# zxhuang1698/ShapeClipper

Measured on AMD Instinct MI355X. Metric: train-step images/sec (Pix3D cfg, bs32/GPU), higher is better.
Workload: dtype f32 (bf16x3-split MFMA, fp32 accumulate)

## Files before the change

### include/shapeclipper_hip.h

```cpp
#ifndef SHAPECLIPPER_HIP_H
#define SHAPECLIPPER_HIP_H
#include <stdint.h>
#ifdef __cplusplus
extern "C" {
#endif

int sc_chamfer3d_forward(const float* xyz1, const float* xyz2, float* dist1, float* dist2,
                         int32_t* idx1, int32_t* idx2, int b, int n, int m, void* stream);

int sc_chamfer3d_forward_split(const float* xyz1, const float* xyz2, float* dist1, float* dist2,
                               int32_t* idx1, int32_t* idx2, int b, int n, int m, int nsplit,
                               void* workspace, void* stream);

long long sc_chamfer3d_grid_workspace_bytes(int b, int n, int m);
int sc_chamfer3d_forward_grid(const float* xyz1, const float* xyz2, float* dist1, float* dist2,
                              int32_t* idx1, int32_t* idx2, int b, int n, int m, void* workspace, void* stream);

int sc_chamfer3d_backward(const float* xyz1, const float* xyz2, float* gradxyz1, float* gradxyz2,
                          const float* graddist1, const float* graddist2, const int32_t* idx1,
                          const int32_t* idx2, int b, int n, int m, void* stream);

long long sc_chamfer3d_backward_ordered_workspace_bytes(int b, int n, int m);
int sc_chamfer3d_backward_ordered_chunk(void);
int sc_chamfer3d_backward_ordered(const float* xyz1, const float* xyz2, float* gradxyz1, float* gradxyz2,
// ... 372 lines not shown

long long sc_conv3x3s2_bd_pack_floats(int cin, int cout, int hw);
long long sc_conv3x3s2_bd_workspace_floats(int hw);
int sc_conv3x3s2_bd_pack(const float* w, float* w_pack, int cin, int cout, int hw, void* stream);
int sc_conv3x3s2_backward_data(const float* gy, const float* w_pack, float* gx, float* workspace, int batch, int cin, int cout, int hw,
                               void* stream);
int sc_conv3x3s2_wgrad(const float* gy, const float* x, float* dw, float* workspace, int batch, int cin, int cout, int hw, void* stream);
long long sc_conv3x3s2_pack_floats(int cin, int cout, int hw);
long long sc_conv3x3s2_workspace_floats(int hw);
int sc_conv3x3s2_forward(const float* x, const float* w_pack, float* out, float* workspace, int batch, int cin, int cout, int hw,
                         void* stream);

long long sc_conv3x3_wgrad_workspace_floats(int cin, int cout);
int sc_conv3x3_wgrad(const float* gy, const float* x, float* dw, float* workspace, int batch, int cin, int cout, int hw, void* stream);
int sc_conv3x3_wgrad_split(const float* gy, const float* x, float* dw, float* workspace, int batch, int cin, int cout, int hw, void* stream);

long long sc_conv_stem_wgrad_workspace_floats(void);
int sc_conv_stem_forward(const float* x, const float* w, float* out, int batch, void* stream);
int sc_conv_stem_wgrad(const float* gy, const float* x, float* dw, float* workspace, int batch, void* stream);

long long sc_conv1x1s2_wgrad_workspace_floats(int cin, int cout);
int sc_conv1x1s2_forward(const float* x, const float* w, float* out, int batch, int cin, int cout, int hin, void* stream);
int sc_conv1x1s2_backward_data(const float* gy, const float* w, float* gx, int batch, int cin, int cout, int hin, void* stream);
int sc_conv1x1s2_wgrad(const float* gy, const float* x, float* dw, float* workspace, int batch, int cin, int cout, int hin, void* stream);

typedef struct sc_block_args {
    const float *x, *pf1, *pf2, *pb1, *pb2;
    const float *g1, *b1, *g2, *b2;
    float *rm1, *rv1, *rm2, *rv2;
    int64_t *nt1, *nt2;
// ... 57 lines not shown
```

### shapeclipper_amd/_lib.py

```python
from __future__ import annotations

import ctypes
import os
import re
import threading
from typing import Optional

import torch

_HERE = os.path.dirname(os.path.abspath(__file__))
LIB_PATH = os.environ.get("SHAPECLIPPER_HIP_LIB") or os.path.join(_HERE, "lib", "libshapeclipper_hip.so")

HEADER_PATH = os.path.join(_HERE, os.pardir, "include", "shapeclipper_hip.h")
_CTYPES = {"int": ctypes.c_int, "long long": ctypes.c_longlong, "float": ctypes.c_float, "double": ctypes.c_double}


def read_signatures(text):
    text = re.sub(r"/\*.*?\*/|//[^\n]*", " ", text, flags=re.S)
    text = re.sub(r"^[ \t]*#.*$", " ", text, flags=re.M)
    text = re.sub(r"typedef struct sc_block_args \{.*?\} sc_block_args", " ", text, flags=re.S)
    text = re.sub(r'extern "C" \{|\}', " ", text)
    sigs = {}
    for decl in filter(None, (" ".join(d.split()) for d in text.split(";"))):
        m = re.fullmatch(r"(int|long long) (sc_\w+)\((.*)\)", decl)
        if m is None:
            raise RuntimeError("shapeclipper_amd: include/shapeclipper_hip.h: unrecognised declaration %r" % decl)
        params = [] if m.group(3) == "void" else m.group(3).split(",")
        try:
            args = [ctypes.c_void_p if "*" in p else _CTYPES[" ".join(w for w in p.split()[:-1] if w != "const")] for p in params]
        except KeyError:
            raise RuntimeError("shapeclipper_amd: include/shapeclipper_hip.h: unrecognised parameter type in %r" % decl) from None
        sigs[m.group(2)] = (_CTYPES[m.group(1)], args)
    return sigs


with open(HEADER_PATH) as _f:
    SIGNATURES = read_signatures(_f.read())
SYMBOLS = tuple(n for n, (res, _) in SIGNATURES.items() if res is ctypes.c_int)
SYMBOLS_OTHER = tuple(n for n, (res, _) in SIGNATURES.items() if res is ctypes.c_longlong)

_lib: Optional[ctypes.CDLL] = None

TIMING = None
TIMING_SKIP = ("sc_sdf_stream_pack", "sc_sdf_stream_pack_bytes", "sc_rgb_composite_backward_fused_parts", "sc_rgb_composite_backward_fused_partial_floats", "sc_latent_bias_forward", "sc_latent_bias_backward", "sc_set_reserved_cus", "sc_grid_cus", "sc_chamfer3d_backward_ordered_chunk","sc_conv3x3_release_tables", "sc_linear_bn_supported", "sc_linear_bn_forward", "sc_linear_bn_backward", "sc_linear_backward_data", "sc_bn_splits", "sc_isosurface_blocks_per_image", "sc_marching_cubes_mesh_vertex_blocks_per_image", "sc_bn_act_forward", "sc_bn_act_backward", "sc_bn_relu_pool_forward", "sc_bn_relu_pool_backward",
               "sc_conv3x3_forward", "sc_conv3x3_forward_split", "sc_conv3x3_forward_add", "sc_conv3x3_wgrad", "sc_conv3x3_wgrad_split", "sc_conv3x3_pack", "sc_conv3x3_pack_multi", "sc_conv3x3_pack_multi_units",
               "sc_conv_stem_forward", "sc_conv_stem_wgrad", "sc_conv1x1s2_forward", "sc_conv1x1s2_backward_data", "sc_conv1x1s2_wgrad",
               "sc_conv3x3s2_forward", "sc_conv3x3s2_bd_pack", "sc_conv3x3s2_backward_data", "sc_conv3x3s2_wgrad", "sc_conv3x3_tile_channels", "sc_conv3x3_tile_channels_split",
               "sc_basic_block_forward", "sc_basic_block_backward")

class _Timed:

    def __init__(self, name, fn):
        self.name, self.fn = name, fn

    def __call__(self, *args):
        if TIMING is None:
            return self.fn(*args)
        s, e = torch.cuda.Event(enable_timing=True), torch.cuda.Event(enable_timing=True)
        s.record()
        code = self.fn(*args)
# ... 64 lines not shown
```

### shapeclipper_amd/csrc/block.hip

```cpp
#include <hip/hip_runtime.h>
#include <stdint.h>

#include "shapeclipper_hip.h"


extern "C" int sc_basic_block_forward(const sc_block_args* a, void* stream) {
    if (!a || a->batch <= 0 || a->channels <= 0) return (int)hipErrorInvalidValue;
    const int B = a->batch, C = a->channels, hw = a->hw, HW = hw * hw, G = a->groups;
    auto conv = a->split ? sc_conv3x3_forward_split : sc_conv3x3_forward;
    int rc = conv(a->x, a->pf1, a->y1, a->conv_ws, B, C, C, hw, stream);
    if (rc) return rc;
    rc = sc_bn_act_forward(a->y1, nullptr, a->g1, a->b1, a->a1, a->st1, a->st1 + (size_t)G * C, a->rm1, a->rv1, a->nt1, a->bn_ws, B, C, HW, 1,
                           a->training, G, a->eps1, a->mom1, stream);
    if (rc) return rc;
    rc = conv(a->a1, a->pf2, a->y2, a->conv_ws, B, C, C, hw, stream);
    if (rc) return rc;
    return sc_bn_act_forward(a->y2, a->x, a->g2, a->b2, a->out, a->st2, a->st2 + (size_t)G * C, a->rm2, a->rv2, a->nt2, a->bn_ws, B, C, HW, 1,
                             a->training, G, a->eps2, a->mom2, stream);
}

extern "C" int sc_basic_block_backward(const sc_block_args* a, void* stream) {
    if (!a || a->batch <= 0 || a->channels <= 0 || !a->d_out) return (int)hipErrorInvalidValue;
    const int B = a->batch, C = a->channels, hw = a->hw, HW = hw * hw, G = a->groups;
    auto conv = a->split ? sc_conv3x3_forward_split : sc_conv3x3_forward;
    auto wgrad = a->split ? sc_conv3x3_wgrad_split : sc_conv3x3_wgrad;
    int rc = sc_bn_act_backward(a->d_out, a->y2, a->out, a->g2, a->b2, a->st2, a->st2 + (size_t)G * C, a->bn_ws, a->dy2, a->need_dx ? a->dres : nullptr,
                                a->dgb2, a->dgb2 + C, B, C, HW, 1, a->training, G, stream);
    if (rc) return rc;
    rc = conv(a->dy2, a->pb2, a->da1, a->conv_ws, B, C, C, hw, stream);
    if (rc) return rc;
    if (a->gw2) {
        rc = wgrad(a->dy2, a->a1, a->gw2, a->wgrad_ws, B, C, C, hw, stream);
        if (rc) return rc;
    }
    rc = sc_bn_act_backward(a->da1, a->y1, nullptr, a->g1, a->b1, a->st1, a->st1 + (size_t)G * C, a->bn_ws, a->dy1, nullptr, a->dgb1, a->dgb1 + C, B,
                            C, HW, 1, a->training, G, stream);
    if (rc) return rc;
    if (a->need_dx) {
        rc = sc_conv3x3_forward_add(a->dy1, a->pb1, a->dres, a->dx, a->conv_ws, B, C, C, hw, a->split, stream);
        if (rc) return rc;
    }
    if (a->gw1) rc = wgrad(a->dy1, a->x, a->gw1, a->wgrad_ws, B, C, C, hw, stream);
    return rc;
}
```

### shapeclipper_amd/csrc/conv3x3_wgrad.hip

```cpp
#include <hip/hip_runtime.h>

#include "grid_cus.hpp"
#include "shapeclipper_hip.h"

namespace sc {

typedef float wg_f32x16 __attribute__((ext_vector_type(16)));

#ifdef SC_WGRAD_PROFILE
__device__ unsigned long long* wgrad_prof_buf = nullptr;
#define WG_STAMP(ID) { const unsigned long long t_ = __builtin_amdgcn_s_memrealtime(); if (wgrad_prof_buf && tid == 0) wgrad_prof_buf[(size_t)blockIdx.x * 16 + (ID)] = t_; }
#define WG_ACCUM(ID, T0) { const unsigned long long t_ = __builtin_amdgcn_s_memrealtime(); if (wgrad_prof_buf && tid == 0) wgrad_prof_buf[(size_t)blockIdx.x * 16 + (ID)] += t_ - (T0); }
#else
#define WG_STAMP(ID)
#endif

template <int W_, int NR_, int NIMG_, int GS_, int S_ = 1>
struct WgCfg {
    static constexpr int W = W_, H = W_, NR = NR_, NIMG = NIMG_, GS = GS_, S = S_;
    static constexpr int HW = W * W;
    static constexpr int XW = S * W, XH = S * H, XHW = XW * XH;
    static constexpr int Wp = S == 1 ? W + 2 : XW + 1;
    static constexpr bool WHOLE = NR == H;
    static constexpr int SLOTW = (W + 2 * GS - 1) / (2 * GS) * (2 * GS);
// ... 147 lines not shown
            for (int t = 0; t < 3; ++t)
#pragma unroll
                for (int r = 0; r < 16; ++r) acc[pass * 3 + t][r] += R[((wt * 3 + t) * 16 + r) * 64 + lane];
        }
        __syncthreads();
    }
    if (kh == 0) {
        float* dst = partial + (size_t)blockIdx.x * (64 * 64 * 9);
#pragma unroll
        for (int t = 0; t < 9; ++t)
#pragma unroll
            for (int r = 0; r < 16; ++r) dst[((wt * 9 + t) * 16 + r) * 64 + lane] = acc[t][r];
    }
}

__global__ __launch_bounds__(256) void conv3x3_wgrad_reduce_kernel(const float* __restrict__ partial, float* __restrict__ dw, int cin,
                                                                  int cout, int S) {
    __shared__ float part[4][64];
    const int nti = cin / 64, lane = threadIdx.x & 63, w = threadIdx.x >> 6;
    const int blk = blockIdx.x / 576, e = (blockIdx.x - blk * 576) * 64 + lane;
    const float* src = partial + (size_t)blk * S * 36864 + e;
    float s0 = 0.f, s1 = 0.f;
    int s = w;
    for (; s + 4 < S; s += 8) {
        s0 += src[(size_t)s * 36864];
        s1 += src[(size_t)(s + 4) * 36864];
    }
    if (s < S) s0 += src[(size_t)s * 36864];
    part[w][lane] = s0 + s1;
    __syncthreads();
    if (w == 0) {
        const float sum = (part[0][lane] + part[1][lane]) + (part[2][lane] + part[3][lane]);
        const int r = (e >> 6) & 15, t = (e >> 10) % 9, wt = e / (9 * 1024);
        const int co = (blk / nti) * 64 + (wt >> 1) * 32 + (r & 3) + 8 * (r >> 2) + 4 * (lane >> 5);
        const int ci = (blk % nti) * 64 + (wt & 1) * 32 + (lane & 31);
        dw[((size_t)co * cin + ci) * 9 + t] = sum;
// ... 24 lines not shown
    static constexpr int BSTR = (PATCH + 3) / 4 * 4 + 2;
    static constexpr bool WHOLE = NR == H;
    static constexpr int LDS_BYTES = 3 * 64 * (ASTR + BSTR) * 2;
    static constexpr int CHUNK = W == 7 ? 49 : 56, RPC = CHUNK / W;
    static constexpr int XROWS = WHOLE ? H : PR;
    static constexpr int XCH = (XROWS + RPC - 1) / RPC, GCH = (NR + RPC - 1) / RPC;
    static_assert(NSLOT % 16 == 0 && H % NR == 0 && LDS_BYTES <= 160 * 1024 && (W >= 14 || (NIMG == 2 && NR == 7)), "K-step shape");
    static constexpr int boff(int g, int h) {
        if (W == 7) { const int r = 2 * g + h; return ((r / 7) * PR + r % 7) * Wp; }
        const int r = g / (SLOTS / 16), gx = g % (SLOTS / 16);
        return ((r / NR) * PR + r % NR) * Wp + 16 * gx + 8 * h;
    }
};

template <class C>
__global__ __launch_bounds__(768, 1) void conv3x3_wgrad_split_kernel(const float* __restrict__ gy, const float* __restrict__ x,
                                                                     float* __restrict__ partial, int batch, int cin, int cout, int S) {
    constexpr int W = C::W, H = C::H, HW = C::HW, Wp = C::Wp, NIMG = C::NIMG, NR = C::NR;
    extern __shared__ float4 wg_smem[];
    __bf16* As = reinterpret_cast<__bf16*>(wg_smem);
    __bf16* Xs = As + 3 * 64 * C::ASTR;
    const int tid = threadIdx.x, lane = tid & 63, wave = __builtin_amdgcn_readfirstlane(tid >> 6), half = lane >> 5;
    const int wt = wave & 3, ky = wave >> 2;
    const int nti = cin / 64;
    const int blk = blockIdx.x / S, s = blockIdx.x - blk * S;
    const int co0 = (blk / nti) * 64, ci0 = (blk % nti) * 64;
    const int nimg_steps = NIMG == 2 ? (batch + 1) / 2 : batch * (H / NR);
    const int k_lo = (int)((long long)s * nimg_steps / S), k_hi = (int)((long long)(s + 1) * nimg_steps / S);

    for (int i = tid; i < C::LDS_BYTES / 16; i += 768) wg_smem[i] = make_float4(0.f, 0.f, 0.f, 0.f);

    const bool lane_on = lane < C::CHUNK, xrole = wave < 8;
    const int lrow = lane / W, lx = lane - lrow * W;
    constexpr int NSV = 8 * C::XCH * NIMG > 16 * C::GCH * NIMG ? 8 * C::XCH * NIMG : 16 * C::GCH * NIMG;
    float sv[NSV];
    auto load = [&](int kstep) {
        int b, y0;
        if (NIMG == 2) { b = 2 * kstep; y0 = 0; } else { b = kstep / (H / NR); y0 = (kstep - b * (H / NR)) * NR; }
        if (xrole) {
#pragma unroll
            for (int im = 0; im < NIMG; ++im) {
                const float* xb = x + ((size_t)(b + im) * cin + ci0 + 8 * wave) * HW;
#pragma unroll
                for (int c = 0; c < C::XCH; ++c) {
                    const int rr = c * C::RPC + lrow, yr = (C::WHOLE ? 0 : y0 - 1) + rr;
                    const bool ok = lane_on && b + im < batch && (unsigned)yr < (unsigned)H && rr < C::XROWS;
                    const int off = yr * W + lx;
#pragma unroll
                    for (int ch = 0; ch < 8; ++ch) sv[(im * C::XCH + c) * 8 + ch] = ok ? xb[ch * HW + off] : 0.f;
                }
// ... 37 lines not shown
            for (int im = 0; im < NIMG; ++im)
#pragma unroll
                for (int c = 0; c < C::GCH; ++c) {
                    const int rr = c * C::RPC + lrow;
                    if (lane_on && rr < NR) {
                        __bf16* d = As + 16 * (wave - 8) * C::ASTR + (im * NR + rr) * C::SLOTS + lx;
#pragma unroll
                        for (int ch = 0; ch < 16; ++ch) put(d + ch * C::ASTR, 64 * C::ASTR, sv[(im * C::GCH + c) * 16 + ch]);
                    }
                }
        }
    };

#if SC_WGRAD_S16
    wg_f32x4 acc[3][2][2];
#pragma unroll
    for (int t = 0; t < 3; ++t)
#pragma unroll
        for (int u = 0; u < 4; ++u) acc[t][u >> 1][u & 1] = wg_f32x4{0.f, 0.f, 0.f, 0.f};
    const int q4 = lane >> 4, l16 = lane & 15;
    const __bf16* Ab = As + ((wt >> 1) * 32 + l16) * C::ASTR + 8 * q4;
    const unsigned* Bb = reinterpret_cast<const unsigned*>(Xs + ((wt & 1) * 32 + l16) * C::BSTR + ky * Wp);
#else
    wg_f32x16 acc[3];
#pragma unroll
    for (int t = 0; t < 3; ++t)
#pragma unroll
        for (int r = 0; r < 16; ++r) acc[t][r] = 0.f;

    const __bf16* Ab = As + ((wt >> 1) * 32 + (lane & 31)) * C::ASTR + 8 * half;
    const unsigned* Bb = reinterpret_cast<const unsigned*>(Xs + ((wt & 1) * 32 + (lane & 31)) * C::BSTR + ky * Wp);
#endif

    WG_STAMP(0)
    if (k_lo < k_hi) load(k_lo);
    __syncthreads();
    WG_STAMP(1)
    for (int kstep = k_lo; kstep < k_hi; ++kstep) {
#ifdef SC_WGRAD_PROFILE
        const unsigned long long ts0 = __builtin_amdgcn_s_memrealtime();
#endif
        store();
        __syncthreads();
#ifdef SC_WGRAD_PROFILE
        WG_ACCUM(4, ts0)
        const unsigned long long ts1 = __builtin_amdgcn_s_memrealtime();
#endif
        if (kstep + 1 < k_hi) load(kstep + 1);
#if SC_WGRAD_S16
#pragma unroll
        for (int G2 = 0; G2 < (C::G + 1) / 2; ++G2) {
            constexpr int NG = C::G;
            const bool tail = 2 * G2 + 1 >= NG;
            const bool dead = tail && q4 >= 2;
            const int g1 = tail ? 2 * G2 : 2 * G2 + 1;
            const int bo = (q4 == 0 ? C::boff(2 * G2, 0) : q4 == 1 ? C::boff(2 * G2, 1) : q4 == 2 ? C::boff(g1, 0) : C::boff(g1, 1)) >> 1;
            float4 a[3][2];
#pragma unroll
            for (int pc = 0; pc < 3; ++pc)
#pragma unroll
                for (int u = 0; u < 2; ++u) {
                    const float4 av = *reinterpret_cast<const float4*>(Ab + pc * 64 * C::ASTR + u * 16 * C::ASTR + (dead ? 0 : 32 * G2));
                    a[pc][u] = dead ? make_float4(0.f, 0.f, 0.f, 0.f) : av;
                }
#pragma unroll
            for (int sb = 0; sb < 2; ++sb) {
                unsigned d[3][5];
#pragma unroll
                for (int pc = 0; pc < 3; ++pc)
#pragma unroll
                    for (int q = 0; q < 5; ++q) d[pc][q] = Bb[pc * 32 * C::BSTR + sb * 8 * C::BSTR + bo + q];
#pragma unroll
                for (int term = 0; term < 6; ++term) {
                    constexpr int PA[6] = {0, 2, 1, 0, 1, 0}, PB[6] = {2, 0, 1, 1, 0, 0};
                    const unsigned* q = d[PB[term]];
                    const uint4 b0 = {q[0], q[1], q[2], q[3]}, b2 = {q[1], q[2], q[3], q[4]};
                    const uint4 b1 = {__builtin_amdgcn_alignbit(q[1], q[0], 16), __builtin_amdgcn_alignbit(q[2], q[1], 16),
                                      __builtin_amdgcn_alignbit(q[3], q[2], 16), __builtin_amdgcn_alignbit(q[4], q[3], 16)};
#pragma unroll
                    for (int sa = 0; sa < 2; ++sa) {
                        const wg_bf16x8 av = __builtin_bit_cast(wg_bf16x8, a[PA[term]][sa]);
                        acc[0][sa][sb] = __builtin_amdgcn_mfma_f32_16x16x32_bf16(av, __builtin_bit_cast(wg_bf16x8, b0), acc[0][sa][sb], 0, 0, 0);
                        acc[1][sa][sb] = __builtin_amdgcn_mfma_f32_16x16x32_bf16(av, __builtin_bit_cast(wg_bf16x8, b1), acc[1][sa][sb], 0, 0, 0);
                        acc[2][sa][sb] = __builtin_amdgcn_mfma_f32_16x16x32_bf16(av, __builtin_bit_cast(wg_bf16x8, b2), acc[2][sa][sb], 0, 0, 0);
                    }
                }
#pragma unroll
                for (int pc = 0; pc < 3; ++pc)
                    asm volatile("" : "+v"(acc[0][0][sb]) : "v"(d[pc][0]), "v"(d[pc][1]), "v"(d[pc][2]), "v"(d[pc][3]), "v"(d[pc][4]));
            }
#pragma unroll
            for (int pc = 0; pc < 3; ++pc)
                asm volatile("" : "+v"(acc[0][0][0]) : "v"(__builtin_bit_cast(wg_f32x4, a[pc][0])), "v"(__builtin_bit_cast(wg_f32x4, a[pc][1])));
            __builtin_amdgcn_sched_barrier(0);
        }
#else
#pragma unroll
        for (int g = 0; g < C::G; ++g) {
            float4 a[3];
            unsigned d[3][5];
            const int bo = (half ? C::boff(g, 1) : C::boff(g, 0)) >> 1;
#pragma unroll
            for (int pc = 0; pc < 3; ++pc) {
                a[pc] = *reinterpret_cast<const float4*>(Ab + pc * 64 * C::ASTR + 16 * g);
#pragma unroll
                for (int q = 0; q < 5; ++q) d[pc][q] = Bb[pc * 32 * C::BSTR + bo + q];
            }
#pragma unroll
            for (int term = 0; term < 6; ++term) {
                constexpr int PA[6] = {0, 2, 1, 0, 1, 0}, PB[6] = {2, 0, 1, 1, 0, 0};
                const unsigned* q = d[PB[term]];
                const wg_bf16x8 av = __builtin_bit_cast(wg_bf16x8, a[PA[term]]);
                uint4 b0 = {q[0], q[1], q[2], q[3]}, b2 = {q[1], q[2], q[3], q[4]};
                uint4 b1 = {__builtin_amdgcn_alignbit(q[1], q[0], 16), __builtin_amdgcn_alignbit(q[2], q[1], 16),
                            __builtin_amdgcn_alignbit(q[3], q[2], 16), __builtin_amdgcn_alignbit(q[4], q[3], 16)};
                acc[0] = __builtin_amdgcn_mfma_f32_32x32x16_bf16(av, __builtin_bit_cast(wg_bf16x8, b0), acc[0], 0, 0, 0);
                acc[1] = __builtin_amdgcn_mfma_f32_32x32x16_bf16(av, __builtin_bit_cast(wg_bf16x8, b1), acc[1], 0, 0, 0);
                acc[2] = __builtin_amdgcn_mfma_f32_32x32x16_bf16(av, __builtin_bit_cast(wg_bf16x8, b2), acc[2], 0, 0, 0);
            }
        }
#endif
        __syncthreads();
#ifdef SC_WGRAD_PROFILE
        WG_ACCUM(5, ts1)
#endif
    }
    WG_STAMP(2)
    float* dst = partial + (size_t)blockIdx.x * (64 * 64 * 9);
#if SC_WGRAD_S16
#pragma unroll
    for (int t = 0; t < 3; ++t)
#pragma unroll
        for (int sa = 0; sa < 2; ++sa)
#pragma unroll
            for (int sb = 0; sb < 2; ++sb)
#pragma unroll
                for (int r = 0; r < 4; ++r)
                    dst[((wt * 9 + ky * 3 + t) * 16 + r + 4 * (2 * sa + (q4 >> 1))) * 64 + 16 * sb + l16 + 32 * (q4 & 1)] = acc[t][sa][sb][r];
#else
#pragma unroll
    for (int t = 0; t < 3; ++t)
#pragma unroll
        for (int r = 0; r < 16; ++r) dst[((wt * 9 + ky * 3 + t) * 16 + r) * 64 + lane] = acc[t][r];
#endif
#ifdef SC_WGRAD_PROFILE
    asm volatile("s_waitcnt vmcnt(0)" ::: "memory");
    WG_STAMP(3)
    if (wgrad_prof_buf && tid == 0) wgrad_prof_buf[(size_t)blockIdx.x * 16 + 6] = (unsigned long long)(k_hi - k_lo);
#endif
}

using Ws56 = WsCfg<56, 2, 1>;
using Ws28 = WsCfg<28, 4, 1>;
using Ws14 = WsCfg<14, 7, 1>;
using Ws7 = WsCfg<7, 7, 2>;

static int wg_cus() { return grid_cus(); }
static int wg_splits(int cin, int cout) {
    const int nblk = (cin / 64) * (cout / 64), s = wg_cus() / nblk;
    return s > 0 ? s : 1;
}

template <class C>
static int launch_wgrad(const float* gy, const float* x, float* dw, float* workspace, int batch, int cin, int cout, hipStream_t st) {
    if (cin % 64 || cout % 64 || batch <= 0) return (int)hipErrorInvalidValue;
    const int nblk = (cin / 64) * (cout / 64), S = wg_splits(cin, cout);
    (void)hipFuncSetAttribute((const void*)conv3x3_wgrad_kernel<C>, hipFuncAttributeMaxDynamicSharedMemorySize, C::LDS_FLOATS * 4);
    hipLaunchKernelGGL((conv3x3_wgrad_kernel<C>), dim3(nblk * S), dim3(512), C::LDS_FLOATS * 4, st, gy, x, workspace, batch, cin, cout, S);
    hipLaunchKernelGGL(conv3x3_wgrad_reduce_kernel, dim3(nblk * 576), dim3(256), 0, st, workspace, dw, cin, cout, S);
    return (int)hipGetLastError();
}

template <class C>
static int launch_wgrad_split(const float* gy, const float* x, float* dw, float* workspace, int batch, int cin, int cout, hipStream_t st) {
    if (cin % 64 || cout % 64 || batch <= 0) return (int)hipErrorInvalidValue;
    const int nblk = (cin / 64) * (cout / 64), S = wg_splits(cin, cout);
    (void)hipFuncSetAttribute((const void*)conv3x3_wgrad_split_kernel<C>, hipFuncAttributeMaxDynamicSharedMemorySize, C::LDS_BYTES);
    hipLaunchKernelGGL((conv3x3_wgrad_split_kernel<C>), dim3(nblk * S), dim3(768), C::LDS_BYTES, st, gy, x, workspace, batch, cin, cout, S);
    hipLaunchKernelGGL(conv3x3_wgrad_reduce_kernel, dim3(nblk * 576), dim3(256), 0, st, workspace, dw, cin, cout, S);
    return (int)hipGetLastError();
}

}

#ifdef SC_WGRAD_PROFILE
extern "C" int sc_wgrad_debug_set_prof(unsigned long long* buf) {
    return (int)hipMemcpyToSymbol(HIP_SYMBOL(sc::wgrad_prof_buf), &buf, sizeof(buf));
}
#endif
extern "C" int sc_conv3x3_wgrad_split(const float* gy, const float* x, float* dw, float* workspace, int batch, int cin, int cout, int hw, void* stream) {
    switch (hw) {
        case 56: return sc::launch_wgrad_split<sc::Ws56>(gy, x, dw, workspace, batch, cin, cout, (hipStream_t)stream);
        case 28: return sc::launch_wgrad_split<sc::Ws28>(gy, x, dw, workspace, batch, cin, cout, (hipStream_t)stream);
        case 14: return sc::launch_wgrad_split<sc::Ws14>(gy, x, dw, workspace, batch, cin, cout, (hipStream_t)stream);
        case 7: return sc::launch_wgrad_split<sc::Ws7>(gy, x, dw, workspace, batch, cin, cout, (hipStream_t)stream);
        default: return -1;
    }
}

extern "C" long long sc_conv3x3_wgrad_workspace_floats(int cin, int cout) {
    if (cin <= 0 || cout <= 0 || cin % 64 || cout % 64) return -1;
    return (long long)(cin / 64) * (cout / 64) * sc::wg_splits(cin, cout) * 36864;
}

extern "C" int sc_conv3x3s2_wgrad(const float* gy, const float* x, float* dw, float* workspace, int batch, int cin, int cout, int hw, void* stream) {
    switch (hw) {
        case 56: return sc::launch_wgrad<sc::Wg28S2>(gy, x, dw, workspace, batch, cin, cout, (hipStream_t)stream);
        case 28: return sc::launch_wgrad<sc::Wg14S2>(gy, x, dw, workspace, batch, cin, cout, (hipStream_t)stream);
        case 14: return sc::launch_wgrad<sc::Wg7S2>(gy, x, dw, workspace, batch, cin, cout, (hipStream_t)stream);
        default: return -1;
    }
}

extern "C" int sc_conv3x3_wgrad(const float* gy, const float* x, float* dw, float* workspace, int batch, int cin, int cout, int hw, void* stream) {
    switch (hw) {
        case 56: return sc::launch_wgrad<sc::Wg56>(gy, x, dw, workspace, batch, cin, cout, (hipStream_t)stream);
        case 28: return sc::launch_wgrad<sc::Wg28>(gy, x, dw, workspace, batch, cin, cout, (hipStream_t)stream);
// ... 6 lines not shown
```

### shapeclipper_amd/ops.py

```python
from __future__ import annotations

import collections
import ctypes
import weakref

import torch

from . import _lib
from .packing import n_tiles

_SCRATCH = {}


def _scratch(tag, dev, n_floats):
    if dev.type != "cuda":
        raise RuntimeError(_lib.NO_CPU)
    key = (tag, dev.index, torch._C._cuda_getCurrentRawStream(dev.index))
    buf = _SCRATCH.get(key)
    if buf is None or buf.numel() < n_floats:
        buf = _SCRATCH[key] = torch.empty(n_floats, device=dev, dtype=torch.float32)
    return buf


SDF_SCRATCH_FLOATS = 256 * 8 * 5 * 1024
# ... 979 lines not shown
def conv3x3_backward_weight(gy, x, split=False):
    lib = _lib.load()
    gy, x = _aligned(gy), _aligned(x)
    B, cout, H, _ = gy.shape
    cin = x.shape[1]
    n = lib.sc_conv3x3_wgrad_workspace_floats(cin, cout)
    if n < 0 or H not in CONV3X3_SIDES or x.shape[0] != B or tuple(x.shape[2:]) != (H, H):
        raise RuntimeError("shapeclipper_amd: sc_conv3x3_wgrad does not take gy %s with x %s" % (tuple(gy.shape), tuple(x.shape)))
    ws = _scratch("conv wgrad", x.device, n)
    dw = torch.empty(cout, cin, 3, 3, device=x.device, dtype=torch.float32)
    fn = lib.sc_conv3x3_wgrad_split if split else lib.sc_conv3x3_wgrad
    _lib.check(fn(_lib.ptr(gy), _lib.ptr(x), _lib.ptr(dw), _lib.ptr(ws), B, cin, cout, H, _lib.stream()), "sc_conv3x3_wgrad")
    return dw


class BlockArgs(ctypes.Structure):
    _fields_ = ([(n, ctypes.c_void_p) for n in ("x", "pf1", "pf2", "pb1", "pb2", "g1", "b1", "g2", "b2", "rm1", "rv1", "rm2", "rv2", "nt1", "nt2",
                                   "y1", "a1", "y2", "out", "st1", "st2", "conv_ws", "bn_ws", "wgrad_ws", "d_out",
                                   "dy2", "dres", "da1", "dy1", "dx", "gw1", "gw2", "dgb1", "dgb2")]
                + [(n, ctypes.c_int) for n in ("batch", "channels", "hw", "groups", "training", "split", "need_dx")]
                + [(n, ctypes.c_float) for n in ("mom1", "eps1", "mom2", "eps2")])


def _wgrad_workspace(x, cin, cout):
    return _scratch("conv wgrad", x.device, _lib.load().sc_conv3x3_wgrad_workspace_floats(cin, cout))


def basic_block_forward(x, pf1, pf2, g1, b1, g2, b2, bn1_state, bn2_state, split, groups):
    B, C, H, _ = x.shape
    rm1, rv1, nt1, training, mom1, eps1 = bn1_state
    rm2, rv2, nt2, _, mom2, eps2 = bn2_state
    y1, a1, y2, out = (torch.empty_like(x) for _ in range(4))
    st = torch.empty(2, 2, groups, C, device=x.device, dtype=torch.float32)
    a = BlockArgs()
    a.x, a.pf1, a.pf2 = x.data_ptr(), pf1.data_ptr(), pf2.data_ptr()
    a.g1, a.b1, a.g2, a.b2 = g1.data_ptr(), b1.data_ptr(), g2.data_ptr(), b2.data_ptr()
    a.rm1, a.rv1, a.nt1, a.rm2, a.rv2, a.nt2 = _p(rm1), _p(rv1), _p(nt1), _p(rm2), _p(rv2), _p(nt2)
    a.y1, a.a1, a.y2, a.out = y1.data_ptr(), a1.data_ptr(), y2.data_ptr(), out.data_ptr()
    a.st1, a.st2 = st[0].data_ptr(), st[1].data_ptr()
    a.conv_ws, a.bn_ws = _conv_workspace(x.device, H, split).data_ptr(), _bn_partial(x, groups)
# ... 8 lines not shown
def basic_block_backward(d_out, x, saved, out, pb1, pb2, g1, b1, g2, b2, training, split, groups, need_dx, need_w1, need_w2):
    y1, a1, y2, st1, st2 = saved
    B, C, H, _ = x.shape
    dy2, da1, dy1 = (torch.empty_like(x) for _ in range(3))
    dx, dres = (torch.empty_like(x), torch.empty_like(x)) if need_dx else (None, None)
    gw1 = torch.empty(C, C, 3, 3, device=x.device, dtype=torch.float32) if need_w1 else None
    gw2 = torch.empty(C, C, 3, 3, device=x.device, dtype=torch.float32) if need_w2 else None
    dgb = torch.empty(2, 2, C, device=x.device, dtype=torch.float32)
    a = BlockArgs()
    a.x, a.pb1, a.pb2, a.d_out = x.data_ptr(), pb1.data_ptr(), pb2.data_ptr(), d_out.data_ptr()
    a.g1, a.b1, a.g2, a.b2 = g1.data_ptr(), b1.data_ptr(), g2.data_ptr(), b2.data_ptr()
    a.y1, a.a1, a.y2, a.out, a.st1, a.st2 = y1.data_ptr(), a1.data_ptr(), y2.data_ptr(), out.data_ptr(), st1.data_ptr(), st2.data_ptr()
    a.dy2, a.da1, a.dy1, a.dres, a.dx = dy2.data_ptr(), da1.data_ptr(), dy1.data_ptr(), _p(dres), _p(dx)
    a.gw1, a.gw2, a.dgb1, a.dgb2 = _p(gw1), _p(gw2), dgb[0].data_ptr(), dgb[1].data_ptr()
    a.conv_ws, a.bn_ws = _conv_workspace(x.device, H, split).data_ptr(), _bn_partial(x, groups)
    a.wgrad_ws = _wgrad_workspace(x, C, C).data_ptr() if (need_w1 or need_w2) else None
    a.batch, a.channels, a.hw, a.groups, a.training, a.split, a.need_dx = B, C, H, groups, 1 if training else 0, 1 if split else 0, 1 if need_dx else 0
    code = _lib.load().sc_basic_block_backward(ctypes.byref(a), _lib.raw_stream(x.get_device()))
    if code:
        _lib.check(code, "sc_basic_block_backward")
    return dx, gw1, dgb[0, 0], dgb[0, 1], gw2, dgb[1, 0], dgb[1, 1]


def conv_stem_supported(x_shape, w_shape, stride=2, padding=3) -> bool:
    return (tuple(x_shape[1:]) == (3, 224, 224) and tuple(w_shape) == (64, 3, 7, 7) and stride in (2, (2, 2)) and padding in (3, (3, 3)))


def conv_stem_forward(x, w):
    lib = _lib.load()
    x, w = _aligned(x), _aligned(w)
    out = torch.empty(x.shape[0], 64, 112, 112, device=x.device, dtype=torch.float32)
# ... 632 lines not shown
```

Measured before the change: 1035.

## Batch both basic-block weight-gradient convolutions into one multi-job wgrad launch

The residual block backward now defers both 3x3 weight-gradient computations to the end and, on the split path, runs them in a single persistent kernel that loops over up to four jobs, prefetching the next job's first tile while writing partials. A single reduce kernel then handles all jobs' partials. This removes one pair of kernel launches and the per-kernel ramp-up and tail per block, at the cost of a larger workspace (two jobs' partials) and a longer single kernel that runs after the data-gradient convolution rather than interleaved with it.

Result: slower. 1007 (-2.8%).

```diff
diff --git a/include/shapeclipper_hip.h b/include/shapeclipper_hip.h
--- a/include/shapeclipper_hip.h
+++ b/include/shapeclipper_hip.h
@@ -410,6 +410,14 @@
 long long sc_conv3x3_wgrad_workspace_floats(int cin, int cout);
 int sc_conv3x3_wgrad(const float* gy, const float* x, float* dw, float* workspace, int batch, int cin, int cout, int hw, void* stream);
 int sc_conv3x3_wgrad_split(const float* gy, const float* x, float* dw, float* workspace, int batch, int cin, int cout, int hw, void* stream);
+#define SC_WGRAD_MAX_JOBS 4
+typedef struct sc_wgrad_job {
+    const float* gy;
+    const float* x;
+    float* dw;
+} sc_wgrad_job;
+long long sc_conv3x3_wgrad_multi_workspace_floats(int cin, int cout, int n);
+int sc_conv3x3_wgrad_split_multi(const sc_wgrad_job* jobs, int n, float* workspace, int batch, int cin, int cout, int hw, void* stream);
 
 long long sc_conv_stem_wgrad_workspace_floats(void);
 int sc_conv_stem_forward(const float* x, const float* w, float* out, int batch, void* stream);
diff --git a/shapeclipper_amd/_lib.py b/shapeclipper_amd/_lib.py
--- a/shapeclipper_amd/_lib.py
+++ b/shapeclipper_amd/_lib.py
@@ -18,7 +18,7 @@
 def read_signatures(text):
     text = re.sub(r"/\*.*?\*/|//[^\n]*", " ", text, flags=re.S)
     text = re.sub(r"^[ \t]*#.*$", " ", text, flags=re.M)
-    text = re.sub(r"typedef struct sc_block_args \{.*?\} sc_block_args", " ", text, flags=re.S)
+    text = re.sub(r"typedef struct (sc_\w+) \{.*?\} \1", " ", text, flags=re.S)
     text = re.sub(r'extern "C" \{|\}', " ", text)
     sigs = {}
     for decl in filter(None, (" ".join(d.split()) for d in text.split(";"))):
@@ -43,7 +43,7 @@
 
 TIMING = None
 TIMING_SKIP = ("sc_sdf_stream_pack", "sc_sdf_stream_pack_bytes", "sc_rgb_composite_backward_fused_parts", "sc_rgb_composite_backward_fused_partial_floats", "sc_latent_bias_forward", "sc_latent_bias_backward", "sc_set_reserved_cus", "sc_grid_cus", "sc_chamfer3d_backward_ordered_chunk","sc_conv3x3_release_tables", "sc_linear_bn_supported", "sc_linear_bn_forward", "sc_linear_bn_backward", "sc_linear_backward_data", "sc_bn_splits", "sc_isosurface_blocks_per_image", "sc_marching_cubes_mesh_vertex_blocks_per_image", "sc_bn_act_forward", "sc_bn_act_backward", "sc_bn_relu_pool_forward", "sc_bn_relu_pool_backward",
-               "sc_conv3x3_forward", "sc_conv3x3_forward_split", "sc_conv3x3_forward_add", "sc_conv3x3_wgrad", "sc_conv3x3_wgrad_split", "sc_conv3x3_pack", "sc_conv3x3_pack_multi", "sc_conv3x3_pack_multi_units",
+               "sc_conv3x3_forward", "sc_conv3x3_forward_split", "sc_conv3x3_forward_add", "sc_conv3x3_wgrad", "sc_conv3x3_wgrad_split", "sc_conv3x3_wgrad_split_multi", "sc_conv3x3_pack", "sc_conv3x3_pack_multi", "sc_conv3x3_pack_multi_units",
                "sc_conv_stem_forward", "sc_conv_stem_wgrad", "sc_conv1x1s2_forward", "sc_conv1x1s2_backward_data", "sc_conv1x1s2_wgrad",
                "sc_conv3x3s2_forward", "sc_conv3x3s2_bd_pack", "sc_conv3x3s2_backward_data", "sc_conv3x3s2_wgrad", "sc_conv3x3_tile_channels", "sc_conv3x3_tile_channels_split",
                "sc_basic_block_forward", "sc_basic_block_backward")
diff --git a/shapeclipper_amd/csrc/block.hip b/shapeclipper_amd/csrc/block.hip
--- a/shapeclipper_amd/csrc/block.hip
+++ b/shapeclipper_amd/csrc/block.hip
@@ -23,16 +23,11 @@
     if (!a || a->batch <= 0 || a->channels <= 0 || !a->d_out) return (int)hipErrorInvalidValue;
     const int B = a->batch, C = a->channels, hw = a->hw, HW = hw * hw, G = a->groups;
     auto conv = a->split ? sc_conv3x3_forward_split : sc_conv3x3_forward;
-    auto wgrad = a->split ? sc_conv3x3_wgrad_split : sc_conv3x3_wgrad;
     int rc = sc_bn_act_backward(a->d_out, a->y2, a->out, a->g2, a->b2, a->st2, a->st2 + (size_t)G * C, a->bn_ws, a->dy2, a->need_dx ? a->dres : nullptr,
                                 a->dgb2, a->dgb2 + C, B, C, HW, 1, a->training, G, stream);
     if (rc) return rc;
     rc = conv(a->dy2, a->pb2, a->da1, a->conv_ws, B, C, C, hw, stream);
     if (rc) return rc;
-    if (a->gw2) {
-        rc = wgrad(a->dy2, a->a1, a->gw2, a->wgrad_ws, B, C, C, hw, stream);
-        if (rc) return rc;
-    }
     rc = sc_bn_act_backward(a->da1, a->y1, nullptr, a->g1, a->b1, a->st1, a->st1 + (size_t)G * C, a->bn_ws, a->dy1, nullptr, a->dgb1, a->dgb1 + C, B,
                             C, HW, 1, a->training, G, stream);
     if (rc) return rc;
@@ -40,6 +35,15 @@
         rc = sc_conv3x3_forward_add(a->dy1, a->pb1, a->dres, a->dx, a->conv_ws, B, C, C, hw, a->split, stream);
         if (rc) return rc;
     }
-    if (a->gw1) rc = wgrad(a->dy1, a->x, a->gw1, a->wgrad_ws, B, C, C, hw, stream);
-    return rc;
+    sc_wgrad_job jobs[2];
+    int n = 0;
+    if (a->gw2) jobs[n++] = {a->dy2, a->a1, a->gw2};
+    if (a->gw1) jobs[n++] = {a->dy1, a->x, a->gw1};
+    if (n == 0) return 0;
+    if (a->split) return sc_conv3x3_wgrad_split_multi(jobs, n, a->wgrad_ws, B, C, C, hw, stream);
+    for (int j = 0; j < n; ++j) {
+        rc = sc_conv3x3_wgrad(jobs[j].gy, jobs[j].x, jobs[j].dw, a->wgrad_ws, B, C, C, hw, stream);
+        if (rc) return rc;
+    }
+    return 0;
 }
diff --git a/shapeclipper_amd/csrc/conv3x3_wgrad.hip b/shapeclipper_amd/csrc/conv3x3_wgrad.hip
--- a/shapeclipper_amd/csrc/conv3x3_wgrad.hip
+++ b/shapeclipper_amd/csrc/conv3x3_wgrad.hip
@@ -6,6 +6,10 @@
 namespace sc {
 
 typedef float wg_f32x16 __attribute__((ext_vector_type(16)));
+
+struct WgJobs {
+    sc_wgrad_job j[SC_WGRAD_MAX_JOBS];
+};
 
 #ifdef SC_WGRAD_PROFILE
 __device__ unsigned long long* wgrad_prof_buf = nullptr;
@@ -185,12 +189,14 @@
     }
 }
 
-__global__ __launch_bounds__(256) void conv3x3_wgrad_reduce_kernel(const float* __restrict__ partial, float* __restrict__ dw, int cin,
-                                                                  int cout, int S) {
+__global__ __launch_bounds__(256) void conv3x3_wgrad_reduce_kernel(const float* __restrict__ partial, const WgJobs jobs, int cin, int cout,
+                                                                  int S) {
     __shared__ float part[4][64];
-    const int nti = cin / 64, lane = threadIdx.x & 63, w = threadIdx.x >> 6;
-    const int blk = blockIdx.x / 576, e = (blockIdx.x - blk * 576) * 64 + lane;
-    const float* src = partial + (size_t)blk * S * 36864 + e;
+    const int nti = cin / 64, nblk = nti * (cout / 64), lane = threadIdx.x & 63, w = threadIdx.x >> 6;
+    const int job = blockIdx.x / (nblk * 576), bj = blockIdx.x - job * (nblk * 576);
+    const int blk = bj / 576, e = (bj - blk * 576) * 64 + lane;
+    const float* src = partial + ((size_t)job * nblk + blk) * S * 36864 + e;
+    float* __restrict__ dw = jobs.j[job].dw;
     float s0 = 0.f, s1 = 0.f;
     int s = w;
     for (; s + 4 < S; s += 8) {
@@ -245,8 +251,8 @@
 };
 
 template <class C>
-__global__ __launch_bounds__(768, 1) void conv3x3_wgrad_split_kernel(const float* __restrict__ gy, const float* __restrict__ x,
-                                                                     float* __restrict__ partial, int batch, int cin, int cout, int S) {
+__global__ __launch_bounds__(768, 1) void conv3x3_wgrad_split_kernel(const WgJobs jobs, int njobs, float* __restrict__ partial, int batch,
+                                                                     int cin, int cout, int S) {
     constexpr int W = C::W, H = C::H, HW = C::HW, Wp = C::Wp, NIMG = C::NIMG, NR = C::NR;
     extern __shared__ float4 wg_smem[];
     __bf16* As = reinterpret_cast<__bf16*>(wg_smem);
@@ -265,6 +271,8 @@
     const int lrow = lane / W, lx = lane - lrow * W;
     constexpr int NSV = 8 * C::XCH * NIMG > 16 * C::GCH * NIMG ? 8 * C::XCH * NIMG : 16 * C::GCH * NIMG;
     float sv[NSV];
+    const float* gy = jobs.j[0].gy;
+    const float* x = jobs.j[0].x;
     auto load = [&](int kstep) {
         int b, y0;
         if (NIMG == 2) { b = 2 * kstep; y0 = 0; } else { b = kstep / (H / NR); y0 = (kstep - b * (H / NR)) * NR; }
@@ -332,20 +340,11 @@
 
 #if SC_WGRAD_S16
     wg_f32x4 acc[3][2][2];
-#pragma unroll
-    for (int t = 0; t < 3; ++t)
-#pragma unroll
-        for (int u = 0; u < 4; ++u) acc[t][u >> 1][u & 1] = wg_f32x4{0.f, 0.f, 0.f, 0.f};
     const int q4 = lane >> 4, l16 = lane & 15;
     const __bf16* Ab = As + ((wt >> 1) * 32 + l16) * C::ASTR + 8 * q4;
     const unsigned* Bb = reinterpret_cast<const unsigned*>(Xs + ((wt & 1) * 32 + l16) * C::BSTR + ky * Wp);
 #else
     wg_f32x16 acc[3];
-#pragma unroll
-    for (int t = 0; t < 3; ++t)
-#pragma unroll
-        for (int r = 0; r < 16; ++r) acc[t][r] = 0.f;
-
     const __bf16* Ab = As + ((wt >> 1) * 32 + (lane & 31)) * C::ASTR + 8 * half;
     const unsigned* Bb = reinterpret_cast<const unsigned*>(Xs + ((wt & 1) * 32 + (lane & 31)) * C::BSTR + ky * Wp);
 #endif
@@ -354,113 +353,131 @@
     if (k_lo < k_hi) load(k_lo);
     __syncthreads();
     WG_STAMP(1)
-    for (int kstep = k_lo; kstep < k_hi; ++kstep) {
+    for (int job = 0; job < njobs; ++job) {
+#if SC_WGRAD_S16
+#pragma unroll
+        for (int t = 0; t < 3; ++t)
+#pragma unroll
+            for (int u = 0; u < 4; ++u) acc[t][u >> 1][u & 1] = wg_f32x4{0.f, 0.f, 0.f, 0.f};
+#else
+#pragma unroll
+        for (int t = 0; t < 3; ++t)
+#pragma unroll
+            for (int r = 0; r < 16; ++r) acc[t][r] = 0.f;
+#endif
+        for (int kstep = k_lo; kstep < k_hi; ++kstep) {
 #ifdef SC_WGRAD_PROFILE
-        const unsigned long long ts0 = __builtin_amdgcn_s_memrealtime();
-#endif
-        store();
-        __syncthreads();
+            const unsigned long long ts0 = __builtin_amdgcn_s_memrealtime();
+#endif
+            store();
+            __syncthreads();
 #ifdef SC_WGRAD_PROFILE
-        WG_ACCUM(4, ts0)
-        const unsigned long long ts1 = __builtin_amdgcn_s_memrealtime();
-#endif
-        if (kstep + 1 < k_hi) load(kstep + 1);
+            WG_ACCUM(4, ts0)
+            const unsigned long long ts1 = __builtin_amdgcn_s_memrealtime();
+#endif
+            if (kstep + 1 < k_hi) load(kstep + 1);
 #if SC_WGRAD_S16
 #pragma unroll
-        for (int G2 = 0; G2 < (C::G + 1) / 2; ++G2) {
-            constexpr int NG = C::G;
-            const bool tail = 2 * G2 + 1 >= NG;
-            const bool dead = tail && q4 >= 2;
-            const int g1 = tail ? 2 * G2 : 2 * G2 + 1;
-            const int bo = (q4 == 0 ? C::boff(2 * G2, 0) : q4 == 1 ? C::boff(2 * G2, 1) : q4 == 2 ? C::boff(g1, 0) : C::boff(g1, 1)) >> 1;
-            float4 a[3][2];
-#pragma unroll
-            for (int pc = 0; pc < 3; ++pc)
-#pragma unroll
-                for (int u = 0; u < 2; ++u) {
-                    const float4 av = *reinterpret_cast<const float4*>(Ab + pc * 64 * C::ASTR + u * 16 * C::ASTR + (dead ? 0 : 32 * G2));
-                    a[pc][u] = dead ? make_float4(0.f, 0.f, 0.f, 0.f) : av;
-                }
-#pragma unroll
-            for (int sb = 0; sb < 2; ++sb) {
+            for (int G2 = 0; G2 < (C::G + 1) / 2; ++G2) {
+                constexpr int NG = C::G;
+                const bool tail = 2 * G2 + 1 >= NG;
+                const bool dead = tail && q4 >= 2;
+                const int g1 = tail ? 2 * G2 : 2 * G2 + 1;
+                const int bo = (q4 == 0 ? C::boff(2 * G2, 0) : q4 == 1 ? C::boff(2 * G2, 1) : q4 == 2 ? C::boff(g1, 0) : C::boff(g1, 1)) >> 1;
+                float4 a[3][2];
+#pragma unroll
+                for (int pc = 0; pc < 3; ++pc)
+#pragma unroll
+                    for (int u = 0; u < 2; ++u) {
+                        const float4 av = *reinterpret_cast<const float4*>(Ab + pc * 64 * C::ASTR + u * 16 * C::ASTR + (dead ? 0 : 32 * G2));
+                        a[pc][u] = dead ? make_float4(0.f, 0.f, 0.f, 0.f) : av;
+                    }
+#pragma unroll
+                for (int sb = 0; sb < 2; ++sb) {
+                    unsigned d[3][5];
+#pragma unroll
+                    for (int pc = 0; pc < 3; ++pc)
+#pragma unroll
+                        for (int q = 0; q < 5; ++q) d[pc][q] = Bb[pc * 32 * C::BSTR + sb * 8 * C::BSTR + bo + q];
+#pragma unroll
+                    for (int term = 0; term < 6; ++term) {
+                        constexpr int PA[6] = {0, 2, 1, 0, 1, 0}, PB[6] = {2, 0, 1, 1, 0, 0};
+                        const unsigned* q = d[PB[term]];
+                        const uint4 b0 = {q[0], q[1], q[2], q[3]}, b2 = {q[1], q[2], q[3], q[4]};
+                        const uint4 b1 = {__builtin_amdgcn_alignbit(q[1], q[0], 16), __builtin_amdgcn_alignbit(q[2], q[1], 16),
+                                          __builtin_amdgcn_alignbit(q[3], q[2], 16), __builtin_amdgcn_alignbit(q[4], q[3], 16)};
+#pragma unroll
+                        for (int sa = 0; sa < 2; ++sa) {
+                            const wg_bf16x8 av = __builtin_bit_cast(wg_bf16x8, a[PA[term]][sa]);
+                            acc[0][sa][sb] = __builtin_amdgcn_mfma_f32_16x16x32_bf16(av, __builtin_bit_cast(wg_bf16x8, b0), acc[0][sa][sb], 0, 0, 0);
+                            acc[1][sa][sb] = __builtin_amdgcn_mfma_f32_16x16x32_bf16(av, __builtin_bit_cast(wg_bf16x8, b1), acc[1][sa][sb], 0, 0, 0);
+                            acc[2][sa][sb] = __builtin_amdgcn_mfma_f32_16x16x32_bf16(av, __builtin_bit_cast(wg_bf16x8, b2), acc[2][sa][sb], 0, 0, 0);
+                        }
+                    }
+#pragma unroll
+                    for (int pc = 0; pc < 3; ++pc)
+                        asm volatile("" : "+v"(acc[0][0][sb]) : "v"(d[pc][0]), "v"(d[pc][1]), "v"(d[pc][2]), "v"(d[pc][3]), "v"(d[pc][4]));
+                }
+#pragma unroll
+                for (int pc = 0; pc < 3; ++pc)
+                    asm volatile("" : "+v"(acc[0][0][0]) : "v"(__builtin_bit_cast(wg_f32x4, a[pc][0])), "v"(__builtin_bit_cast(wg_f32x4, a[pc][1])));
+                __builtin_amdgcn_sched_barrier(0);
+            }
+#else
+#pragma unroll
+            for (int g = 0; g < C::G; ++g) {
+                float4 a[3];
                 unsigned d[3][5];
-#pragma unroll
-                for (int pc = 0; pc < 3; ++pc)
-#pragma unroll
-                    for (int q = 0; q < 5; ++q) d[pc][q] = Bb[pc * 32 * C::BSTR + sb * 8 * C::BSTR + bo + q];
+                const int bo = (half ? C::boff(g, 1) : C::boff(g, 0)) >> 1;
+#pragma unroll
+                for (int pc = 0; pc < 3; ++pc) {
+                    a[pc] = *reinterpret_cast<const float4*>(Ab + pc * 64 * C::ASTR + 16 * g);
+#pragma unroll
+                    for (int q = 0; q < 5; ++q) d[pc][q] = Bb[pc * 32 * C::BSTR + bo + q];
+                }
 #pragma unroll
                 for (int term = 0; term < 6; ++term) {
                     constexpr int PA[6] = {0, 2, 1, 0, 1, 0}, PB[6] = {2, 0, 1, 1, 0, 0};
                     const unsigned* q = d[PB[term]];
-                    const uint4 b0 = {q[0], q[1], q[2], q[3]}, b2 = {q[1], q[2], q[3], q[4]};
-                    const uint4 b1 = {__builtin_amdgcn_alignbit(q[1], q[0], 16), __builtin_amdgcn_alignbit(q[2], q[1], 16),
-                                      __builtin_amdgcn_alignbit(q[3], q[2], 16), __builtin_amdgcn_alignbit(q[4], q[3], 16)};
-#pragma unroll
-                    for (int sa = 0; sa < 2; ++sa) {
-                        const wg_bf16x8 av = __builtin_bit_cast(wg_bf16x8, a[PA[term]][sa]);
-                        acc[0][sa][sb] = __builtin_amdgcn_mfma_f32_16x16x32_bf16(av, __builtin_bit_cast(wg_bf16x8, b0), acc[0][sa][sb], 0, 0, 0);
-                        acc[1][sa][sb] = __builtin_amdgcn_mfma_f32_16x16x32_bf16(av, __builtin_bit_cast(wg_bf16x8, b1), acc[1][sa][sb], 0, 0, 0);
-                        acc[2][sa][sb] = __builtin_amdgcn_mfma_f32_16x16x32_bf16(av, __builtin_bit_cast(wg_bf16x8, b2), acc[2][sa][sb], 0, 0, 0);
-                    }
-                }
-#pragma unroll
-                for (int pc = 0; pc < 3; ++pc)
-                    asm volatile("" : "+v"(acc[0][0][sb]) : "v"(d[pc][0]), "v"(d[pc][1]), "v"(d[pc][2]), "v"(d[pc][3]), "v"(d[pc][4]));
-            }
-#pragma unroll
-            for (int pc = 0; pc < 3; ++pc)
-                asm volatile("" : "+v"(acc[0][0][0]) : "v"(__builtin_bit_cast(wg_f32x4, a[pc][0])), "v"(__builtin_bit_cast(wg_f32x4, a[pc][1])));
-            __builtin_amdgcn_sched_barrier(0);
-        }
+                    const wg_bf16x8 av = __builtin_bit_cast(wg_bf16x8, a[PA[term]]);
+                    uint4 b0 = {q[0], q[1], q[2], q[3]}, b2 = {q[1], q[2], q[3], q[4]};
+                    uint4 b1 = {__builtin_amdgcn_alignbit(q[1], q[0], 16), __builtin_amdgcn_alignbit(q[2], q[1], 16),
+                                __builtin_amdgcn_alignbit(q[3], q[2], 16), __builtin_amdgcn_alignbit(q[4], q[3], 16)};
+                    acc[0] = __builtin_amdgcn_mfma_f32_32x32x16_bf16(av, __builtin_bit_cast(wg_bf16x8, b0), acc[0], 0, 0, 0);
+                    acc[1] = __builtin_amdgcn_mfma_f32_32x32x16_bf16(av, __builtin_bit_cast(wg_bf16x8, b1), acc[1], 0, 0, 0);
+                    acc[2] = __builtin_amdgcn_mfma_f32_32x32x16_bf16(av, __builtin_bit_cast(wg_bf16x8, b2), acc[2], 0, 0, 0);
+                }
+            }
+#endif
+            __syncthreads();
+#ifdef SC_WGRAD_PROFILE
+            WG_ACCUM(5, ts1)
+#endif
+        }
+        WG_STAMP(2)
+        if (job + 1 < njobs) {
+            gy = jobs.j[job + 1].gy;
+            x = jobs.j[job + 1].x;
+            if (k_lo < k_hi) load(k_lo);
+        }
+        float* dst = partial + ((size_t)job * gridDim.x + blockIdx.x) * (64 * 64 * 9);
+#if SC_WGRAD_S16
+#pragma unroll
+        for (int t = 0; t < 3; ++t)
+#pragma unroll
+            for (int sa = 0; sa < 2; ++sa)
+#pragma unroll
+                for (int sb = 0; sb < 2; ++sb)
+#pragma unroll
+                    for (int r = 0; r < 4; ++r)
+                        dst[((wt * 9 + ky * 3 + t) * 16 + r + 4 * (2 * sa + (q4 >> 1))) * 64 + 16 * sb + l16 + 32 * (q4 & 1)] = acc[t][sa][sb][r];
 #else
 #pragma unroll
-        for (int g = 0; g < C::G; ++g) {
-            float4 a[3];
-            unsigned d[3][5];
-            const int bo = (half ? C::boff(g, 1) : C::boff(g, 0)) >> 1;
-#pragma unroll
-            for (int pc = 0; pc < 3; ++pc) {
-                a[pc] = *reinterpret_cast<const float4*>(Ab + pc * 64 * C::ASTR + 16 * g);
-#pragma unroll
-                for (int q = 0; q < 5; ++q) d[pc][q] = Bb[pc * 32 * C::BSTR + bo + q];
-            }
-#pragma unroll
-            for (int term = 0; term < 6; ++term) {
-                constexpr int PA[6] = {0, 2, 1, 0, 1, 0}, PB[6] = {2, 0, 1, 1, 0, 0};
-                const unsigned* q = d[PB[term]];
-                const wg_bf16x8 av = __builtin_bit_cast(wg_bf16x8, a[PA[term]]);
-                uint4 b0 = {q[0], q[1], q[2], q[3]}, b2 = {q[1], q[2], q[3], q[4]};
-                uint4 b1 = {__builtin_amdgcn_alignbit(q[1], q[0], 16), __builtin_amdgcn_alignbit(q[2], q[1], 16),
-                            __builtin_amdgcn_alignbit(q[3], q[2], 16), __builtin_amdgcn_alignbit(q[4], q[3], 16)};
-                acc[0] = __builtin_amdgcn_mfma_f32_32x32x16_bf16(av, __builtin_bit_cast(wg_bf16x8, b0), acc[0], 0, 0, 0);
-                acc[1] = __builtin_amdgcn_mfma_f32_32x32x16_bf16(av, __builtin_bit_cast(wg_bf16x8, b1), acc[1], 0, 0, 0);
-                acc[2] = __builtin_amdgcn_mfma_f32_32x32x16_bf16(av, __builtin_bit_cast(wg_bf16x8, b2), acc[2], 0, 0, 0);
-            }
-        }
-#endif
-        __syncthreads();
-#ifdef SC_WGRAD_PROFILE
-        WG_ACCUM(5, ts1)
-#endif
-    }
-    WG_STAMP(2)
-    float* dst = partial + (size_t)blockIdx.x * (64 * 64 * 9);
-#if SC_WGRAD_S16
-#pragma unroll
-    for (int t = 0; t < 3; ++t)
-#pragma unroll
-        for (int sa = 0; sa < 2; ++sa)
-#pragma unroll
-            for (int sb = 0; sb < 2; ++sb)
-#pragma unroll
-                for (int r = 0; r < 4; ++r)
-                    dst[((wt * 9 + ky * 3 + t) * 16 + r + 4 * (2 * sa + (q4 >> 1))) * 64 + 16 * sb + l16 + 32 * (q4 & 1)] = acc[t][sa][sb][r];
-#else
-#pragma unroll
-    for (int t = 0; t < 3; ++t)
-#pragma unroll
-        for (int r = 0; r < 16; ++r) dst[((wt * 9 + ky * 3 + t) * 16 + r) * 64 + lane] = acc[t][r];
-#endif
+        for (int t = 0; t < 3; ++t)
+#pragma unroll
+            for (int r = 0; r < 16; ++r) dst[((wt * 9 + ky * 3 + t) * 16 + r) * 64 + lane] = acc[t][r];
+#endif
+    }
 #ifdef SC_WGRAD_PROFILE
     asm volatile("s_waitcnt vmcnt(0)" ::: "memory");
     WG_STAMP(3)
@@ -485,17 +502,25 @@
     const int nblk = (cin / 64) * (cout / 64), S = wg_splits(cin, cout);
     (void)hipFuncSetAttribute((const void*)conv3x3_wgrad_kernel<C>, hipFuncAttributeMaxDynamicSharedMemorySize, C::LDS_FLOATS * 4);
     hipLaunchKernelGGL((conv3x3_wgrad_kernel<C>), dim3(nblk * S), dim3(512), C::LDS_FLOATS * 4, st, gy, x, workspace, batch, cin, cout, S);
-    hipLaunchKernelGGL(conv3x3_wgrad_reduce_kernel, dim3(nblk * 576), dim3(256), 0, st, workspace, dw, cin, cout, S);
+    WgJobs one = {};
+    one.j[0].dw = dw;
+    hipLaunchKernelGGL(conv3x3_wgrad_reduce_kernel, dim3(nblk * 576), dim3(256), 0, st, workspace, one, cin, cout, S);
     return (int)hipGetLastError();
 }
 
 template <class C>
-static int launch_wgrad_split(const float* gy, const float* x, float* dw, float* workspace, int batch, int cin, int cout, hipStream_t st) {
-    if (cin % 64 || cout % 64 || batch <= 0) return (int)hipErrorInvalidValue;
+static int launch_wgrad_split(const sc_wgrad_job* jobs, int n, float* workspace, int batch, int cin, int cout, hipStream_t st) {
+    if (!jobs || n < 1 || n > SC_WGRAD_MAX_JOBS || !workspace || cin <= 0 || cout <= 0 || cin % 64 || cout % 64 || batch <= 0)
+        return (int)hipErrorInvalidValue;
+    WgJobs table = {};
+    for (int j = 0; j < n; ++j) {
+        if (!jobs[j].gy || !jobs[j].x || !jobs[j].dw) return (int)hipErrorInvalidValue;
+        table.j[j] = jobs[j];
+    }
     const int nblk = (cin / 64) * (cout / 64), S = wg_splits(cin, cout);
     (void)hipFuncSetAttribute((const void*)conv3x3_wgrad_split_kernel<C>, hipFuncAttributeMaxDynamicSharedMemorySize, C::LDS_BYTES);
-    hipLaunchKernelGGL((conv3x3_wgrad_split_kernel<C>), dim3(nblk * S), dim3(768), C::LDS_BYTES, st, gy, x, workspace, batch, cin, cout, S);
-    hipLaunchKernelGGL(conv3x3_wgrad_reduce_kernel, dim3(nblk * 576), dim3(256), 0, st, workspace, dw, cin, cout, S);
+    hipLaunchKernelGGL((conv3x3_wgrad_split_kernel<C>), dim3(nblk * S), dim3(768), C::LDS_BYTES, st, table, n, workspace, batch, cin, cout, S);
+    hipLaunchKernelGGL(conv3x3_wgrad_reduce_kernel, dim3(n * nblk * 576), dim3(256), 0, st, workspace, table, cin, cout, S);
     return (int)hipGetLastError();
 }
 
@@ -506,19 +531,30 @@
     return (int)hipMemcpyToSymbol(HIP_SYMBOL(sc::wgrad_prof_buf), &buf, sizeof(buf));
 }
 #endif
+extern "C" int sc_conv3x3_wgrad_split_multi(const sc_wgrad_job* jobs, int n, float* workspace, int batch, int cin, int cout, int hw, void* stream) {
+    switch (hw) {
+        case 56: return sc::launch_wgrad_split<sc::Ws56>(jobs, n, workspace, batch, cin, cout, (hipStream_t)stream);
+        case 28: return sc::launch_wgrad_split<sc::Ws28>(jobs, n, workspace, batch, cin, cout, (hipStream_t)stream);
+        case 14: return sc::launch_wgrad_split<sc::Ws14>(jobs, n, workspace, batch, cin, cout, (hipStream_t)stream);
+        case 7: return sc::launch_wgrad_split<sc::Ws7>(jobs, n, workspace, batch, cin, cout, (hipStream_t)stream);
+        default: return -1;
+    }
+}
+
 extern "C" int sc_conv3x3_wgrad_split(const float* gy, const float* x, float* dw, float* workspace, int batch, int cin, int cout, int hw, void* stream) {
-    switch (hw) {
-        case 56: return sc::launch_wgrad_split<sc::Ws56>(gy, x, dw, workspace, batch, cin, cout, (hipStream_t)stream);
-        case 28: return sc::launch_wgrad_split<sc::Ws28>(gy, x, dw, workspace, batch, cin, cout, (hipStream_t)stream);
-        case 14: return sc::launch_wgrad_split<sc::Ws14>(gy, x, dw, workspace, batch, cin, cout, (hipStream_t)stream);
-        case 7: return sc::launch_wgrad_split<sc::Ws7>(gy, x, dw, workspace, batch, cin, cout, (hipStream_t)stream);
-        default: return -1;
-    }
+    const sc_wgrad_job job = {gy, x, dw};
+    return sc_conv3x3_wgrad_split_multi(&job, 1, workspace, batch, cin, cout, hw, stream);
 }
 
 extern "C" long long sc_conv3x3_wgrad_workspace_floats(int cin, int cout) {
     if (cin <= 0 || cout <= 0 || cin % 64 || cout % 64) return -1;
     return (long long)(cin / 64) * (cout / 64) * sc::wg_splits(cin, cout) * 36864;
+}
+
+extern "C" long long sc_conv3x3_wgrad_multi_workspace_floats(int cin, int cout, int n) {
+    if (n < 1 || n > SC_WGRAD_MAX_JOBS) return -1;
+    const long long one = sc_conv3x3_wgrad_workspace_floats(cin, cout);
+    return one < 0 ? -1 : n * one;
 }
 
 extern "C" int sc_conv3x3s2_wgrad(const float* gy, const float* x, float* dw, float* workspace, int batch, int cin, int cout, int hw, void* stream) {
diff --git a/shapeclipper_amd/ops.py b/shapeclipper_amd/ops.py
--- a/shapeclipper_amd/ops.py
+++ b/shapeclipper_amd/ops.py
@@ -1017,6 +1017,30 @@
     return dw
 
 
+class WgradJob(ctypes.Structure):
+    _fields_ = [("gy", ctypes.c_void_p), ("x", ctypes.c_void_p), ("dw", ctypes.c_void_p)]
+
+
+def conv3x3_backward_weight_multi(pairs, dws=None, workspace=None):
+    lib = _lib.load()
+    pairs = [(_aligned(gy), _aligned(x)) for gy, x in pairs]
+    n = len(pairs)
+    B, cout, H, _ = pairs[0][0].shape
+    cin = pairs[0][1].shape[1]
+    floats = lib.sc_conv3x3_wgrad_multi_workspace_floats(cin, cout, n)
+    if floats < 0 or H not in CONV3X3_SIDES or any(tuple(gy.shape) != (B, cout, H, H) or tuple(x.shape) != (B, cin, H, H) for gy, x in pairs):
+        raise RuntimeError("shapeclipper_amd: sc_conv3x3_wgrad_split_multi does not take %d jobs of gy %s with x %s"
+                           % (n, tuple(pairs[0][0].shape), tuple(pairs[0][1].shape)))
+    ws = _scratch("conv wgrad", pairs[0][1].device, floats) if workspace is None else workspace
+    if ws.numel() < floats:
+        raise RuntimeError("shapeclipper_amd: sc_conv3x3_wgrad_split_multi needs a workspace of %d floats" % floats)
+    if dws is None:
+        dws = [torch.empty(cout, cin, 3, 3, device=x.device, dtype=torch.float32) for _, x in pairs]
+    jobs = (WgradJob * n)(*[WgradJob(_lib.ptr(gy), _lib.ptr(x), _lib.ptr(dw)) for (gy, x), dw in zip(pairs, dws)])
+    _lib.check(lib.sc_conv3x3_wgrad_split_multi(jobs, n, _lib.ptr(ws), B, cin, cout, H, _lib.stream()), "sc_conv3x3_wgrad_split_multi")
+    return list(dws)
+
+
 class BlockArgs(ctypes.Structure):
     _fields_ = ([(n, ctypes.c_void_p) for n in ("x", "pf1", "pf2", "pb1", "pb2", "g1", "b1", "g2", "b2", "rm1", "rv1", "rm2", "rv2", "nt1", "nt2",
                                    "y1", "a1", "y2", "out", "st1", "st2", "conv_ws", "bn_ws", "wgrad_ws", "d_out",
@@ -1025,8 +1049,8 @@
                 + [(n, ctypes.c_float) for n in ("mom1", "eps1", "mom2", "eps2")])
 
 
-def _wgrad_workspace(x, cin, cout):
-    return _scratch("conv wgrad", x.device, _lib.load().sc_conv3x3_wgrad_workspace_floats(cin, cout))
+def _wgrad_workspace(x, cin, cout, n):
+    return _scratch("conv wgrad", x.device, _lib.load().sc_conv3x3_wgrad_multi_workspace_floats(cin, cout, n))
 
 
 def basic_block_forward(x, pf1, pf2, g1, b1, g2, b2, bn1_state, bn2_state, split, groups):
@@ -1065,7 +1089,7 @@
     a.dy2, a.da1, a.dy1, a.dres, a.dx = dy2.data_ptr(), da1.data_ptr(), dy1.data_ptr(), _p(dres), _p(dx)
     a.gw1, a.gw2, a.dgb1, a.dgb2 = _p(gw1), _p(gw2), dgb[0].data_ptr(), dgb[1].data_ptr()
     a.conv_ws, a.bn_ws = _conv_workspace(x.device, H, split).data_ptr(), _bn_partial(x, groups)
-    a.wgrad_ws = _wgrad_workspace(x, C, C).data_ptr() if (need_w1 or need_w2) else None
+    a.wgrad_ws = _wgrad_workspace(x, C, C, 2).data_ptr() if (need_w1 or need_w2) else None
     a.batch, a.channels, a.hw, a.groups, a.training, a.split, a.need_dx = B, C, H, groups, 1 if training else 0, 1 if split else 0, 1 if need_dx else 0
     code = _lib.load().sc_basic_block_backward(ctypes.byref(a), _lib.raw_stream(x.get_device()))
     if code:
```
